# Nashatyrev/shadow

Hardware: AMD Instinct MI355X
Metric: APSP wall time + source-SSSPs/sec, 10k-vertex GML graph, 1/2/4/8 MI355X (higher is better)
Workload: dtype u32+f32

## Files before the change

include/shadow_routing.h:

```cpp
#ifndef SHADOW_ROUTING_H
#define SHADOW_ROUTING_H

#include <stddef.h>
#include <stdint.h>

#ifdef __cplusplus
extern "C" {
#endif

#define SRG_OK 0
#define SRG_ERR_ARG 1
#define SRG_ERR_NO_EDGE 2
#define SRG_ERR_MULTI_EDGE 3
#define SRG_ERR_UNREACHABLE 4
#define SRG_ERR_LATENCY_RANGE 5
#define SRG_ERR_HIP 6
#define SRG_ERR_OOM 7
#define SRG_ERR_PARSE 8
#define SRG_ERR_RCCL 9
#define SRG_ERR_INTERNAL 10

typedef struct srg_edge_list {
    uint32_t num_vertices;
    uint32_t directed;
// ... 66 lines not shown
#define SRG_OPT_SIMULATE_RANK 6
#define SRG_OPT_FW_TILE 7
#define SRG_OPT_SPARSE_DELTA_DIV 12
#define SRG_OPT_SPARSE_GLOBAL_BITMAPS 14
#define SRG_OPT_FW_SYMMETRIC 17
#define SRG_OPT_D2H_MODE 20
#define SRG_OPT_LOSS_CHUNKS 21
#define SRG_OPT_SCAN_GROUPS 22
#define SRG_OPT_H2D_CODEC 25
#define SRG_OPT_EDGE_SHARD 29
#define SRG_OPT_LATE_LOSS 30
#define SRG_OPT_FW_LINE_SPLIT 31
#define SRG_OPT_FW_STEP 32
#define SRG_OPT_FW_OVERLAP 33
#define SRG_OPT_TEST_FAULT 34
#define SRG_OPT_TABLE_POOL_BYTES 35
#define SRG_OPT_TABLE_POOL_IDLE_BYTES 36
#define SRG_OPT_CREATE_MS_RUNTIME 37
#define SRG_OPT_CREATE_MS_LIBRARY 38
#define SRG_OPT_FW_XCD_ORDER 39
#define SRG_OPT_SCAN_MIRROR 40
#define SRG_OPT_SCAN_MIRRORED 41
#define SRG_OPT_SCAN_MIRROR_CAP 42
int srg_set_option(srg_ctx* ctx, int option, double value);
int srg_get_option(srg_ctx* ctx, int option, double* value);

int srg_compute_shortest_paths(srg_ctx* ctx, const srg_edge_list* graph,
                               const uint32_t* nodes, uint32_t num_nodes,
                               uint64_t* out_latency_ns, float* out_packet_loss,
                               srg_stats* stats, char* errbuf, size_t errlen);

int srg_compute_shortest_paths_device(srg_ctx* ctx, const srg_edge_list* graph_dev,
                                      const uint32_t* nodes_dev, uint32_t num_nodes,
                                      uint64_t* out_latency_ns_dev, float* out_packet_loss_dev,
                                      void* hip_stream, srg_stats* stats,
                                      char* errbuf, size_t errlen);

int srg_get_direct_paths(srg_ctx* ctx, const srg_edge_list* graph,
                         const uint32_t* nodes, uint32_t num_nodes,
                         uint64_t* out_latency_ns, float* out_packet_loss,
                         srg_stats* stats, char* errbuf, size_t errlen);

typedef struct srg_routing_info srg_routing_info;
int srg_routing_info_build(srg_ctx* ctx, const srg_edge_list* graph, const uint32_t* gml_ids, uint32_t num_ids,
                           int use_shortest_paths, srg_routing_info** out, srg_stats* stats,
                           char* errbuf, size_t errlen);
// ... 89 lines not shown
```

shadow_amd/_native.py:

```python
import ctypes
import os

_HERE = os.path.dirname(os.path.abspath(__file__))
LIB_PATH = os.path.join(_HERE, "libshadow_routing.so")

SRG_OK = 0
SRG_ERR_ARG = 1
SRG_ERR_NO_EDGE = 2
SRG_ERR_MULTI_EDGE = 3
SRG_ERR_UNREACHABLE = 4
SRG_ERR_LATENCY_RANGE = 5
SRG_ERR_HIP = 6
SRG_ERR_OOM = 7
SRG_ERR_PARSE = 8
SRG_ERR_RCCL = 9
SRG_ERR_INTERNAL = 10
SRG_ERR_EVENT_ORDER = 11

SRG_PATH_DENSE_U32 = 0
SRG_PATH_DENSE_U64 = 1
SRG_PATH_DIRECT = 2
SRG_PATH_SPARSE_U32 = 3
SRG_PATH_SPARSE_U64 = 4

# ... 5 lines not shown
SRG_OPT_SIMULATE_RANK = 6
SRG_OPT_FW_TILE = 7
SRG_OPT_SPARSE_DELTA_DIV = 12
SRG_OPT_SPARSE_GLOBAL_BITMAPS = 14
SRG_OPT_FW_SYMMETRIC = 17
SRG_OPT_D2H_MODE = 20
SRG_OPT_LOSS_CHUNKS = 21
SRG_OPT_SCAN_GROUPS = 22
SRG_OPT_H2D_CODEC = 25
SRG_OPT_EDGE_SHARD = 29
SRG_OPT_LATE_LOSS = 30
SRG_OPT_FW_LINE_SPLIT = 31
SRG_OPT_FW_STEP = 32
SRG_OPT_FW_OVERLAP = 33
SRG_OPT_TEST_FAULT = 34
SRG_OPT_TABLE_POOL_BYTES = 35
SRG_OPT_TABLE_POOL_IDLE_BYTES = 36
SRG_OPT_CREATE_MS_RUNTIME = 37
SRG_OPT_CREATE_MS_LIBRARY = 38
SRG_OPT_FW_XCD_ORDER = 39
SRG_OPT_SCAN_MIRROR = 40
SRG_OPT_SCAN_MIRRORED = 41
SRG_OPT_SCAN_MIRROR_CAP = 42
SRG_ALGO_AUTO = 0
SRG_ALGO_DENSE = 1
SRG_ALGO_SPARSE = 2
SRG_UNIQUE_ID_BYTES = 128

SRG_SCAN_NONE = 0
SRG_SCAN_SPARSE = 1
SRG_SCAN_DENSE = 2

_u32p = ctypes.POINTER(ctypes.c_uint32)
_u64p = ctypes.POINTER(ctypes.c_uint64)
_f32p = ctypes.POINTER(ctypes.c_float)


class EdgeList(ctypes.Structure):
    _fields_ = [
        ("num_vertices", ctypes.c_uint32),
        ("directed", ctypes.c_uint32),
        ("num_edges", ctypes.c_uint64),
        ("src", ctypes.c_void_p),
        ("dst", ctypes.c_void_p),
        ("latency_ns", ctypes.c_void_p),
        ("packet_loss", ctypes.c_void_p),
# ... 197 lines not shown
```

shadow_amd/csrc/dense.hip.h:

```cpp
template <class K, int T>
bool run_dense(srg_ctx& c, const DevGraph& g, const Plan& pl, const uint32_t* nodes, uint32_t n, uint64_t* out_lat,
               float* out_loss, hipStream_t st, const Prelude& P, srg_stats* stats, HostSink* sink,
               FwOverlap* ov = nullptr) {
    const bool pre = ov && ov->on && ov->ok && ov->ended && sizeof(K) == 4 && T == FwOverlap::T;
    if (sizeof(K) == 8 && c.kout_key) {
        if (!(sink && sink->widen)) fail(SRG_INTERNAL_NEED_U64, "the build needs u64 latency keys: no u32 key table");
        sink->widen = false;
        c.kout_key = nullptr;
        c.kout_diag = nullptr;
    }
    const uint32_t V = g.V;
    const size_t Vp = ((size_t)V + T - 1) / T * T;
    const size_t VV = Vp * Vp;
    const bool multi = c.comm && c.comm->nranks > 1;
    Timer tm(st);
    c.own_row0 = pl.p0;
    c.own_row1 = pl.p1;

    K* W = (K*)c.b_W.get(VV * sizeof(K));
    uint32_t* WL = (uint32_t*)c.b_WL.get(VV * 4);
    K* D = (K*)c.b_D.get(VV * sizeof(K));
    bool wl_late = false;
    if (pre) {
        wl_late = g.late && !g.late->applied;
// ... 285 lines not shown
            HIP_CHECK(hipEventRecord(c.ev_dst, ax));
        }
        const size_t Eb = E_layout + 256;
        uint32_t* cscpos = (uint32_t*)c.b_cscfill.get((size_t)nbTT5 * nK5 * V5_TT * 4);
        K* ent_w = (K*)c.b_entw.get(Eb * sizeof(K));
        uint2* ent_ub = (uint2*)c.b_grpe.get(Eb * 8);
        uint32_t* cscent = (uint32_t*)c.b_cscent.get(std::max<uint64_t>(E_ess, 1) * 4);
        k_v5_cscpos<<<(NT + 255) / 256, 256, 0, st>>>(v5_cnt, cscoff, NT, nK5, cscpos);
        uint2* rec = (uint2*)c.b_entkey.get((Eb + V5_SLACK) * 8);
        {
            const size_t nwaves = (size_t)nw64 * nK5;
            k_v5_fill<K><<<(unsigned)((nwaves * 64 + 255) / 256), 256, 0, st>>>(ess, W, WL, Vp, V, nw64, nK5, v5_cnt,
                                                                                  v5_goff, cscpos, rec, ent_w,
                                                                                  ent_ub, cscent);
        }
        HIP_CHECK(hipGetLastError());
        const size_t lds_rows = loss_rows_lds(V);
        bool mirror = c.scan_mirror && !g.directed && pl.G == 1 && !multi && !simulated && nloc == n && P.ident &&
                      !v5lo && lds_rows <= 150 * 1024;
        const uint32_t scan_groups = c.scan_groups ? (uint32_t)c.scan_groups : mirror ? 4u : 3u;
        const bool interleave = sink_rows && lds_rows <= 150 * 1024 && scan_groups > 1;
        if (interleave) set_lds(k_loss_rows<K, true>, lds_rows);
        uint32_t* PREDK = lds_rows <= 150 * 1024 ? (uint32_t*)c.b_PRED2.get(nmax * Vp * 8) : nullptr;
        auto pack_pred = [&](uint32_t r0, uint32_t r1) {
            const uint32_t nsb = (r1 - r0 + 127) / 128, nt8 = (nbTT5 + 7) / 8;
            k_pred_pack<<<8u * nt8 * nsb, 256, 0, st>>>(PRED, Vp, r0, r1, NT, nbTT5, nsb, ent_ub, (uint2*)PREDK,
                                                        multi_cnt, mirror ? 1u : 0u);
            HIP_CHECK(hipGetLastError());
        };
        auto mirror_rows = [&](uint32_t r0, uint32_t r1) {
            if (r1 <= r0 || r1 <= SB) return;
            const size_t pairs = (size_t)(r1 - r0) * Vp, room = std::min<size_t>(pairs / 2, (size_t)1 << 30);
            const uint32_t cap = (uint32_t)std::min<size_t>(
                room, c.scan_mirror_cap ? (size_t)c.scan_mirror_cap : std::max<size_t>(pairs / 1024, 256));
            uint2* work = (uint2*)(PRED + (size_t)r0 * Vp);
            HIP_CHECK(hipMemsetAsync(mirror_cnt, 0, 4, st));
            const uint32_t nlow = (r1 - 1) / SB * SB;
            k_pred_mirror<<<dim3(nlow / 64, (r1 - r0 + 63) / 64), 256, 0, st>>>((uint2*)PREDK, Vp, r0, r1, V, work, cap,
                                                                               mirror_cnt, multi_cnt);
            k_mirror_slow<K><<<1024, 256, 0, st>>>(work, mirror_cnt, cap, DST, npad, ent_ub, ent_w, cscoff, cscent,
                                                   (uint2*)PREDK, Vp, multi_cnt);
            HIP_CHECK(hipGetLastError());
        };
        std::vector<uint32_t> tri_h;
        if (nloc) HIP_CHECK(hipStreamWaitEvent(st, c.ev_dst, 0));
        for (bool again = nloc != 0; again;) {
            again = false;
            if (interleave) HIP_CHECK(hipMemsetAsync(&P.flags->changed, 0, 4, st));
            const uint32_t inf_check = v5lo ? 0u : 1u;
            const uint32_t nbS5 = (uint32_t)(npad / SB);
            const uint32_t ng = interleave ? std::min<uint32_t>(scan_groups, nbS5) : 1u;
            auto cut = [&](uint32_t q) { return mirror ? scan_group_cut_tri(q, ng, nbS5) : scan_group_cut(q, ng, nbS5); };
            const uint32_t* tri_d = nullptr;
            std::vector<size_t> tri_off(ng + 1, 0);
            if (mirror) {
                tri_h.clear();
                for (uint32_t gi = 0; gi < ng; ++gi) {
                    tri_scan_blocks(cut(gi), cut(gi + 1), nbTT5, tri_h);
                    tri_off[gi + 1] = tri_h.size();
                }
                uint32_t* d = (uint32_t*)c.b_tri.get(std::max<size_t>(tri_h.size(), 1) * 4);
                if (!tri_h.empty()) HIP_CHECK(hipMemcpyAsync(d, tri_h.data(), tri_h.size() * 4, hipMemcpyHostToDevice, st));
                HIP_CHECK(hipMemsetAsync(mirror_cnt, 0, 8, st));
                tri_d = d;
            }
            for (uint32_t gi = 0; gi < ng; ++gi) {
                const uint32_t c0 = cut(gi), c1 = cut(gi + 1);
                if (c1 == c0) continue;
                const uint32_t nblk = mirror ? (uint32_t)(tri_off[gi + 1] - tri_off[gi])
                                             : (nbTT5 + 3) / 4 * ((c1 - c0 + 7) / 8);
                if (nblk)
                    tight_v5<<<8u * 32u * ((nblk + 7) / 8), V5_WAVES * 64, 0, st>>>(
                        DSTs, npad, dsts_bytes, lnodes, nloc, V, NT, nbTT5, c1, nK5, c0, v5_goff,
                        (const uint32_t*)c.b_entkey.get(0), PRED, Vp, inf_check, mirror ? tri_d + tri_off[gi] : nullptr);
                HIP_CHECK(hipGetLastError());
                if (interleave) {
                    const uint32_t r0 = c0 * SB, r1 = std::min<uint32_t>(c1 * SB, nloc);
                    if (r1 <= r0) continue;
                    pack_pred(r0, r1);
                    if (mirror) mirror_rows(r0, r1);
                    k_loss_rows<K, true><<<r1 - r0, 1024, lds_rows, st>>>(PREDK, Vp, V, lnodes, nloc, ent_ub, ent_w,
                                                                   DST, npad, cscoff, cscent, P.selfloss, nodes, n,
                                                                   lpos, out_loss, &P.flags->changed, r0,
                                                                   mirror ? mirror_cnt + 1 : nullptr);
                    HIP_CHECK(hipGetLastError());
                    sink->send_rows(st, out_loss, sink->loss, pl.p0 + r0, r1 - r0, 4);
                }
            }
            if (!PREDK) k_count_multi<<<nloc, kThreads, 0, st>>>(PRED, nloc, V, Vp, multi_cnt);
            HIP_CHECK(hipGetLastError());
            ms_scan += tm.lap();
            if (interleave) {
                sink->loss_sent = true;
                rb_async(c, MS_CHANGED, &P.flags->changed, st);
                if (mirror) rb_async(c, MS_MIRROR, mirror_cnt + 1, st);
                HIP_CHECK(hipStreamSynchronize(st));
                rounds = (int)rb_get<uint32_t>(c, MS_CHANGED);
                loss_written = true;
            } else if (lds_rows <= 150 * 1024) {
                set_lds(k_loss_rows<K, true>, lds_rows);
                HIP_CHECK(hipMemsetAsync(&P.flags->changed, 0, 4, st));
                pack_pred(0, nloc);
                if (mirror) mirror_rows(0, nloc);
                const uint32_t nchunk = std::max<uint32_t>(1, std::min<uint32_t>(c.loss_chunks ? c.loss_chunks : sink_rows ? 8 : 1, nloc));
                for (uint32_t q = 0; q < nchunk; ++q) {
                    const uint32_t r0 = (uint32_t)((uint64_t)nloc * q / nchunk);
                    const uint32_t r1 = (uint32_t)((uint64_t)nloc * (q + 1) / nchunk);
                    if (r1 == r0) continue;
                    k_loss_rows<K, true><<<r1 - r0, 1024, lds_rows, st>>>(PREDK, Vp, V, lnodes, nloc, ent_ub, ent_w,
                                                                   DST, npad, cscoff, cscent, P.selfloss, nodes, n,
                                                                   lpos, out_loss, &P.flags->changed, r0,
                                                                   mirror ? mirror_cnt + 1 : nullptr);
                    HIP_CHECK(hipGetLastError());
                    if (sink_rows) sink->send_rows(st, out_loss, sink->loss, pl.p0 + r0, r1 - r0, 4);
                }
                if (sink_rows) sink->loss_sent = true;
                rb_async(c, MS_CHANGED, &P.flags->changed, st);
                if (mirror) rb_async(c, MS_MIRROR, mirror_cnt + 1, st);
                HIP_CHECK(hipStreamSynchronize(st));
                rounds = (int)rb_get<uint32_t>(c, MS_CHANGED);
                loss_written = true;
            } else {
                float* L0 = (float*)c.b_L0.get(nmax * Vp * 4);
                float* L1 = (float*)c.b_L1.get(nmax * Vp * 4);
                k_fill<float><<<grid_for((size_t)nloc * Vp), kThreads, 0, st>>>(L0, (size_t)nloc * Vp, 1.0f);
// ... 102 lines not shown
```

shadow_amd/csrc/env_switches.h:

```cpp
#pragma once
#include <algorithm>
#include <cstddef>
#include <cstdlib>
#include <cstring>

namespace srg_env {

static inline bool is_set(const char* name) { return std::getenv(name) != nullptr; }
static inline bool first_char_is(const char* name, char ch) {
    const char* e = std::getenv(name);
    return e && e[0] == ch;
}
static inline bool equals(const char* name, const char* value) {
    const char* e = std::getenv(name);
    return e && std::strcmp(e, value) == 0;
}

static inline bool stream_hops_events() { return equals("SRG_STREAM_HOPS", "events"); }
static inline int fw_bulk_q() {
    const char* e = std::getenv("SRG_FW_BULK_Q");
    return !e ? -1 : e[0] == '0' ? 0 : e[0] == '1' ? 1 : -1;
}
static inline bool debug_overlap() { return is_set("SRG_DEBUG_OVERLAP"); }
static inline int debug_sparse() {
    const char* e = std::getenv("SRG_DEBUG_SPARSE");
    return !e ? 0 : e[0] == '2' ? 2 : 1;
}
static inline bool debug_codec() { return is_set("SRG_DEBUG_CODEC"); }
static inline bool debug_create() { return is_set("SRG_DEBUG_CREATE"); }
static inline bool sparse_kernel_bf() { return equals("SRG_SPARSE_KERNEL", "bf"); }
static inline bool sparse_split_off() { return first_char_is("SRG_SPARSE_SPLIT", '0'); }
static inline bool latency_unit_ns() { return equals("SRG_LATENCY_UNIT", "1"); }
static inline int codec_threads() {
    const char* e = std::getenv("SRG_CODEC_THREADS");
    return e ? std::max(1, std::atoi(e)) : 0;
}
static inline bool codec_seq_off() { return equals("SRG_CODEC_SEQ", "0"); }
static inline bool codec_slow_after(size_t& chunk) {
    const char* e = std::getenv("SRG_CODEC_SLOW_AFTER");
    if (e) chunk = (size_t)std::atoll(e);
    return e != nullptr;
}
static inline bool prefault_on() { return !equals("SRG_PREFAULT", "0"); }
static inline bool no_key_d2h() { return is_set("SRG_NO_KEY_D2H"); }
static inline bool create_warm_off() { return first_char_is("SRG_CREATE_WARM", '0'); }

}
```

shadow_amd/csrc/plan.h:

```cpp
#pragma once
#include <algorithm>
#include <cstddef>
#include <cstdint>
#include <vector>

namespace {

struct Plan {
    int G = 1, g = 0, nb = 0, rb0 = 0, rb1 = 0;
    std::vector<int> blk_lo;
    uint32_t p0 = 0, p1 = 0;
    std::vector<uint32_t> lnodes, lpos;
    int owner(int b) const { return (int)(std::upper_bound(blk_lo.begin(), blk_lo.end(), b) - blk_lo.begin()) - 1; }
    bool own(int b) const { return b >= rb0 && b < rb1; }
};

inline void tri_tile_h(int nb, int idx, int& I, int& J) {
    int i = 0;
    while (i + 1 < nb && (i + 1) * nb - (i + 1) * i / 2 <= idx) ++i;
    I = i;
    J = i + (idx - (i * nb - i * (i - 1) / 2));
}

inline Plan make_plan(int G, int g, uint32_t V, int T, const std::vector<uint32_t>& nodes_h) {
// ... 64 lines not shown
        for (uint32_t sg = 0; c0 + 8 * sg < c1; ++sg)
            for (uint32_t tb = 0; 4 * tb < ntiles; ++tb)
                if (std::min(4 * tb + 3, ntiles - 1) >= c0 + 8 * sg) out.push_back(tb | sg << 16);
    while ((out.size() - base) % 8) out.push_back(TRI_PAD);
}

inline uint64_t tri_scan_work(uint32_t c, uint32_t nblocks) { return (uint64_t)c * nblocks - (uint64_t)c * (c ? c - 1 : 0) / 2; }
inline uint32_t scan_group_cut_tri(uint32_t q, uint32_t ng, uint32_t nblocks) {
    if (q == 0) return 0u;
    if (q >= ng) return nblocks;
    const uint32_t last = nblocks ? (nblocks - 1) / 8 * 8 : 0u;
    const bool tail = ng >= 3 && last > 0;
    const uint32_t end = tail ? last : nblocks;
    const uint32_t parts = tail ? ng - 1 : ng;
    if (q >= parts) return end;
    const uint64_t want = tri_scan_work(end, nblocks) / 2;
    uint32_t c = 0;
    while (c < end && tri_scan_work(c, nblocks) < want) ++c;
    const uint32_t half = std::min(end, (c + 4) / 8 * 8);
    if (q == 1) return half;
    return std::min(end, half + ((end - half) * (q - 1) / (parts - 1) + 4) / 8 * 8);
}

}
```

shadow_amd/csrc/routing.hip:

```cpp
#include <hip/hip_runtime.h>
#include <hsa/hsa.h>
#include <hsa/hsa_ext_amd.h>
#include <sys/mman.h>

#include <algorithm>
#include <atomic>
#include <chrono>
#include <cmath>
#include <condition_variable>
#include <deque>
#include <cstdio>
#include <cstdlib>
#include <cstring>
#include <functional>
#include <map>
#include <memory>
#include <mutex>
#include <new>
#include <stdexcept>
#include <string>
#include <thread>
#include <vector>

#include "../../include/shadow_routing.h"
// ... 705 lines not shown
    DevBuf b_cflags, b_tiles, b_tslot;
    uint32_t* fw_timeout = nullptr;
    unsigned char* hbox = nullptr;
    uint32_t* sig[2] = {nullptr, nullptr};
    uint32_t sig_val[2] = {0, 0};
    bool hop_values = false;
    unsigned long long hop_bound_ticks = 200000000ull;
    Event ev_fwreset;
    Event ev_dst;
    int fw_line_split = 0;
    int fw_step = -1;
    DevBuf b_xlb, b_xflags;
    uint32_t xepoch = 0;
    std::vector<Event> ev_ov;
    uint32_t* kout_key = nullptr;
    uint64_t* kout_diag = nullptr;
    DevBuf b_odiag;
    int fw_overlap = 1;
    int fw_xcd_order = 1;
    int scan_mirror = 1;
    int scan_mirrored = 0;
    int scan_mirror_cap = 0;
    DevBuf b_tri;
    int test_fault = 0;
    std::shared_ptr<TablePool> tpool = std::make_shared<TablePool>();
    double ms_create_runtime = 0, ms_create_lib = 0;
    DevBuf b_ek0, b_ek1, b_eh0, b_eh1, b_ei0, b_ei1, b_ehist, b_eoffs, b_ered;
    ~srg_ctx() {
        delete comm;
        for (uint32_t* p : sig)
            if (p) (void)hipFree(p);
        if (h_lring) (void)hipHostFree(h_lring);
        if (hbox) (void)hipHostFree(hbox);
        for (hipStream_t s : {aux_stream, comm_stream, d2h_stream, stream})
            if (s) (void)hipStreamDestroy(s);
        delete pool;
        if (h_ring) (void)hipHostFree(h_ring);
        tpool->close();
    }
};

namespace {

struct LateLoss {
    hipStream_t ls = nullptr;
    std::thread th;
// ... 1068 lines not shown
            begun = true;
        }
        while (next < nb && (next + 1 < nb ? A >= next + 1 : A >= nb - 1)) {
            fw->pivot(next, A);
            if (dbg) pe.push_back(tev(st));
            ++next;
        }
        if (next == nb && !ended) {
            fw->end(ms_xchg);
            ended = true;
        }
    }
};

#include "dense.hip.h"
#include "sparse_run.hip.h"

void compute_device(srg_ctx& c, const DevGraph& g, const uint32_t* nodes, uint32_t n, uint64_t* out_lat,
                    float* out_loss, hipStream_t st, srg_stats* stats, HostSink* sink = nullptr,
                    FwOverlap* ov = nullptr) {
    HIP_CHECK(hipStreamSynchronize(c.aux_stream));
    HIP_CHECK(hipStreamSynchronize(c.comm_stream));
    c.scan_mirrored = 0;
    if (g.V == 0) {
        if (n) fail(SRG_ERR_ARG, "nodes given for an empty graph");
        return;
    }
    const bool ov_fw = ov && ov->on && ov->ok && ov->begun;
    Prelude P = prelude(c, g, nodes, n, ov_fw ? c.comm_stream : st, true);
    if (n == 0) return;
    const uint64_t unit = (P.es.unit > 1 && !srg_env::latency_unit_ns()) ? P.es.unit : 1;
    P.unit = unit;
    const bool pre = ov && ov->on && ov->ok && ov->ended && P.es.max_lat < 0xFFFFFFFFull;
    if (pre) P.unit = 1;
    P.max_key = P.es.max_lat / P.unit;
    if (stats) stats->latency_unit_ns = P.unit;
    const unsigned __int128 bound = (unsigned __int128)P.max_key * (g.V > 1 ? g.V - 1 : 1);
    P.range_risk = bound >= ((unsigned __int128)1 << 62);
    P.wrap_risk = (unsigned __int128)P.es.max_lat * g.V >= ((unsigned __int128)1 << 64);
    const int G = c.comm ? c.comm->nranks : 1, rk = c.comm ? c.comm->rank : 0;
    if (choose_sparse(c, g) && !P.wrap_risk) {
        loss_arrive(g, P.selfloss, st);
        if (P.max_key < 0xFFFFFFFFull && run_sparse(c, g, nodes, n, out_lat, out_loss, st, P, stats)) return;
        run_sparse(c, g, nodes, n, out_lat, out_loss, st, P, stats, true);
        return;
    }
// ... 1008 lines not shown
        case SRG_OPT_FW_OVERLAP:
            if (value != 0 && value != 1) return SRG_ERR_ARG;
            ctx->fw_overlap = (int)value;
            return SRG_OK;
        case SRG_OPT_TEST_FAULT:
            if (value != 0 && value != 1 && value != 2) return SRG_ERR_ARG;
#ifndef SRG_TEST_HOOKS
            if (value != 0) return SRG_ERR_ARG;
#endif
            ctx->test_fault = (int)value;
            return SRG_OK;
        case SRG_OPT_FW_XCD_ORDER:
            if (value != 0 && value != 1) return SRG_ERR_ARG;
            ctx->fw_xcd_order = (int)value;
            return SRG_OK;
        case SRG_OPT_SCAN_MIRROR:
            if (value != 0 && value != 1) return SRG_ERR_ARG;
            ctx->scan_mirror = (int)value;
            return SRG_OK;
        case SRG_OPT_SCAN_MIRROR_CAP:
            if (!(value >= 0 && value <= 1073741824.0)) return SRG_ERR_ARG;
            ctx->scan_mirror_cap = (int)value;
            return SRG_OK;
        case SRG_OPT_TABLE_POOL_BYTES: {
            if (!(value >= 0.0 && value <= 1e15)) return SRG_ERR_ARG;
            std::lock_guard<std::mutex> pl(ctx->tpool->mu);
            ctx->tpool->limit = (size_t)value;
            ctx->tpool->max_idle = 0;
            ctx->tpool->trim_locked(ctx->tpool->limit);
            return SRG_OK;
        }
        case SRG_OPT_ALGORITHM:
            if (value != SRG_ALGO_AUTO && value != SRG_ALGO_DENSE && value != SRG_ALGO_SPARSE) return SRG_ERR_ARG;
            ctx->algorithm = (int)value;
            return SRG_OK;
        default:
            return SRG_ERR_ARG;
    }
}

int srg_get_option(srg_ctx* ctx, int option, double* value) {
    if (!ctx || !value) return SRG_ERR_ARG;
    std::lock_guard<std::mutex> lk(ctx->mu);
    switch (option) {
        case SRG_OPT_PROFILING: *value = ctx->profiling; break;
        case SRG_OPT_SPARSE_THRESHOLD: *value = ctx->sparse_threshold; break;
// ... 10 lines not shown
        case SRG_OPT_H2D_CODEC: *value = ctx->h2d_codec; break;
        case SRG_OPT_EDGE_SHARD: *value = ctx->edge_shard; break;
        case SRG_OPT_LATE_LOSS: *value = ctx->late_loss; break;
        case SRG_OPT_FW_LINE_SPLIT: *value = ctx->fw_line_split; break;
        case SRG_OPT_FW_STEP: *value = ctx->fw_step; break;
        case SRG_OPT_FW_OVERLAP: *value = ctx->fw_overlap; break;
        case SRG_OPT_TEST_FAULT: *value = ctx->test_fault; break;
        case SRG_OPT_TABLE_POOL_BYTES: {
            std::lock_guard<std::mutex> pl(ctx->tpool->mu);
            *value = (double)ctx->tpool->limit;
            break;
        }
        case SRG_OPT_TABLE_POOL_IDLE_BYTES: {
            std::lock_guard<std::mutex> pl(ctx->tpool->mu);
            *value = (double)ctx->tpool->idle_bytes;
            break;
        }
        case SRG_OPT_CREATE_MS_RUNTIME: *value = ctx->ms_create_runtime; break;
        case SRG_OPT_FW_XCD_ORDER: *value = ctx->fw_xcd_order; break;
        case SRG_OPT_CREATE_MS_LIBRARY: *value = ctx->ms_create_lib; break;
        case SRG_OPT_SCAN_MIRROR: *value = ctx->scan_mirror; break;
        case SRG_OPT_SCAN_MIRRORED: *value = ctx->scan_mirrored; break;
        case SRG_OPT_SCAN_MIRROR_CAP: *value = ctx->scan_mirror_cap; break;
        default: return SRG_ERR_ARG;
    }
    return SRG_OK;
}

void srg_destroy(srg_ctx* ctx) {
    if (!ctx) return;
    (void)hipSetDevice(ctx->device);
    {
        std::lock_guard<std::mutex> lk(g_dev_mu);
        --g_dev_ctx[ctx->device];
    }
    delete ctx;
}

int srg_internal_compute_table(srg_ctx* ctx, const srg_edge_list* graph, const uint32_t* nodes, uint32_t num_nodes,
                               int shortest, uint64_t* out_lat, uint32_t* out_key, uint64_t* out_diag, float* out_loss,
                               uint64_t* unit_ns, srg_table* tab_lat, srg_table* tab_loss, srg_stats* stats,
                               char* errbuf, size_t errlen) {
    srg_stats local{};
    srg_stats* st = stats ? stats : &local;
    srg_table* tabs[2] = {tab_lat, tab_loss};
    const int rc = host_entry(ctx, graph, nodes, num_nodes, out_key ? nullptr : out_lat, out_loss, st, errbuf, errlen,
// ... 375 lines not shown
```

shadow_amd/csrc/tight_sparse.hip.h:

```cpp
#pragma once
#include <hip/hip_runtime.h>
#include <stdint.h>

#include "kernels.hip.h"

namespace srg {

template <class K>
__global__ void __launch_bounds__(256) k_ess_mask(const K* __restrict__ W, const K* __restrict__ D, size_t ld,
                                                   uint32_t V, uint32_t u0, uint32_t u1, uint32_t nw64,
                                                   unsigned long long* __restrict__ ess) {
    const uint32_t lane = threadIdx.x & 63, wave = threadIdx.x >> 6;
    const uint32_t u = u0 + blockIdx.x;
    if (u >= u1) return;
    const K* Wu = W + (size_t)u * ld;
    const K* Du = D + (size_t)u * ld;
    unsigned long long* eu = ess + (size_t)u * nw64;
    if constexpr (sizeof(K) == 4) {
        for (uint32_t w0 = wave * 4; w0 < nw64; w0 += 16) {
            const uint32_t t = w0 * 64 + lane * 4;
            uint4 a = make_uint4(0u, 0u, 0u, 0u), d = make_uint4(1u, 1u, 1u, 1u);
            if (t < ld) {
                a = *reinterpret_cast<const uint4*>(Wu + t);
                d = *reinterpret_cast<const uint4*>(Du + t);
// ... 132 lines not shown
            ++e;
        }
    }
    if (c & 1u) {
        rec[e] = make_uint2(0u, KeyOps<uint32_t>::INF);
        ent_w[e] = KeyOps<K>::INF;
        ent_ub[e] = make_uint2(0u, __float_as_uint(1.0f));
    }
    if (j == V5_TW - 1) {
        const uint32_t total = incl;
        for (size_t q = 2 * ((size_t)pbase + total); q < 2 * (size_t)goff[g + 1]; ++q) {
            rec[q] = make_uint2(0u, KeyOps<uint32_t>::INF);
            ent_w[q] = KeyOps<K>::INF;
            ent_ub[q] = make_uint2(0u, __float_as_uint(1.0f));
        }
    }
}

typedef uint32_t v16u_v5 __attribute__((ext_vector_type(16)));
struct alignas(64) V5Grp {
    uint32_t v[16];
};

__global__ void __launch_bounds__(512, 4) tight_v5(const uint32_t* __restrict__ DST, size_t npad, uint32_t dst_bytes,
                                                    const uint32_t* __restrict__ nodes, uint32_t n, uint32_t V,
                                                    uint32_t NT, uint32_t nbTT, uint32_t nbS, uint32_t nK, uint32_t c0,
                                                    const uint32_t* __restrict__ goff, const uint32_t* __restrict__ rec,
                                                    uint32_t* __restrict__ PRED, size_t ldp, uint32_t inf_check,
                                                    const uint32_t* __restrict__ tri) {
    __shared__ __attribute__((aligned(16))) uint32_t rows[2 * V5_UC * V5_SB];
    const uint32_t bid = blockIdx.x, xcd = bid & 7, slot = bid >> 3;
    const uint32_t blk = (slot >> 5) * 8 + xcd, nbb = (nbTT + 3) / 4;
    uint32_t tb = blk % nbb, sg = blk / nbb;
    if (tri) {
        const uint32_t d = tri[blk];
        if (d == 0xFFFFFFFFu) return;
        tb = d & 0xFFFFu;
        sg = d >> 16;
    }
    const uint32_t b = tb * 4 + (slot & 3), c = c0 + sg * 8 + ((slot >> 2) & 7);
    if (c >= nbS || b >= nbTT) return;
    if (tri && b < c) return;
    const uint32_t tid = threadIdx.x, lane = tid & 63;
    const uint32_t wave = (uint32_t)__builtin_amdgcn_readfirstlane(tid >> 6);
    const uint32_t r0 = c * V5_SB + 2 * lane;
    const __amdgpu_buffer_rsrc_t rsrc = make_rsrc(DST, dst_bytes);
    const uint32_t t0 = b * V5_TT + wave * V5_TW;
    const bool active = t0 < NT;
    v16u_v5 ndl, ndh, stl, sth;
#pragma unroll
    for (uint32_t j = 0; j < V5_TW; ++j) {
        uint32_t dl = 0, dh = 0;
        if (active) {
            const auto v = __builtin_amdgcn_raw_buffer_load_b64(rsrc, ((t0 + j) * (uint32_t)npad + r0) * 4u, 0, 0);
            dl = v[0];
            dh = v[1];
        }
        ndl[j] = 0u - dl;
        ndh[j] = 0u - dh;
        stl[j] = PRED_NONE;
        sth[j] = PRED_NONE;
    }
    const uint32_t srow = tid >> 5, scol = (tid & 31) * 4;
    uint4 sv[4];
    auto stage_load = [&](uint32_t k) {
#pragma unroll
        for (uint32_t i = 0; i < 4; ++i) {
            const uint32_t u = k * V5_UC + srow + 16 * i;
            const auto v = __builtin_amdgcn_raw_buffer_load_b128(rsrc, (u * (uint32_t)npad + c * V5_SB + scol) * 4u, 0, 0);
            sv[i] = make_uint4(v[0], v[1], v[2], v[3]);
        }
    };
    auto stage_store = [&](uint32_t buf) {
#pragma unroll
        for (uint32_t i = 0; i < 4; ++i)
            *reinterpret_cast<uint4*>(&rows[buf * (V5_UC * V5_SB) + (srow + 16 * i) * V5_SB + scol]) = sv[i];
    };
    stage_load(0);
    stage_store(0);
    __syncthreads();
    const unsigned char* lds = reinterpret_cast<const unsigned char*>(rows);
    for (uint32_t k = 0; k < nK; ++k) {
        if (k + 1 < nK) stage_load(k + 1);
        if (active) {
            const size_t q = ((size_t)b * nK + k) * V5_WAVES + wave;
            const uint32_t p0 = (uint32_t)__builtin_amdgcn_readfirstlane(goff[q]);
            const uint32_t p1 = (uint32_t)__builtin_amdgcn_readfirstlane(goff[q + 1]);
            const uint32_t vb = (k & 1u) * (V5_UC * V5_SB * 4u) + lane * 8u;
            auto group = [&](const V5Grp& cur, uint32_t p) {
                    uint2 A[8];
#pragma unroll
                    for (uint32_t i = 0; i < 4; ++i) {
                        A[2 * i] = *reinterpret_cast<const uint2*>(lds + vb + (cur.v[4 * i] & 0xFFFFu));
                        A[2 * i + 1] = *reinterpret_cast<const uint2*>(lds + vb + cur.v[4 * i + 2]);
                    }
#pragma unroll
                    for (uint32_t i = 0; i < 4; ++i) {
                        const uint32_t tl = cur.v[4 * i] >> 16;
                        const uint32_t dl = ndl[tl], dh = ndh[tl];
                        const uint32_t w0 = cur.v[4 * i + 1], w1 = cur.v[4 * i + 3];
                        const uint32_t x0l = A[2 * i].x + w0 + dl, x0h = A[2 * i].y + w0 + dh;
                        const uint32_t x1l = A[2 * i + 1].x + w1 + dl, x1h = A[2 * i + 1].y + w1 + dh;
                        const uint32_t m = min(min(x0l, x0h), min(x1l, x1h));
                        if (__builtin_expect(__ballot(m == 0) != 0, 0)) {
                            const uint32_t e0 = 2 * (p + i);
                            uint32_t sl = stl[tl], sh = sth[tl];
                            if (x0l == 0) sl = (sl == PRED_NONE) ? e0 : PRED_MULTI;
                            if (x1l == 0) sl = (sl == PRED_NONE) ? e0 + 1 : PRED_MULTI;
                            if (x0h == 0) sh = (sh == PRED_NONE) ? e0 : PRED_MULTI;
                            if (x1h == 0) sh = (sh == PRED_NONE) ? e0 + 1 : PRED_MULTI;
                            stl[tl] = sl;
                            sth[tl] = sh;
                        }
                    }
            };
            if (p0 < p1) {
                V5Grp ga = *reinterpret_cast<const V5Grp*>(rec + 4 * (size_t)p0);
                V5Grp gb = *reinterpret_cast<const V5Grp*>(rec + 4 * (size_t)(p0 + 4));
                for (uint32_t p = p0;; p += 8) {
                    group(ga, p);
                    if (p + 4 >= p1) break;
                    ga = *reinterpret_cast<const V5Grp*>(rec + 4 * (size_t)(p + 8));
                    group(gb, p + 4);
                    if (p + 8 >= p1) break;
                    gb = *reinterpret_cast<const V5Grp*>(rec + 4 * (size_t)(p + 12));
                }
            }
        }
        if (k + 1 < nK) {
            stage_store((k + 1) & 1u);
            __syncthreads();
        }
    }
    if (!active) return;
#pragma unroll
    for (uint32_t h = 0; h < 2; ++h) {
        const uint32_t r = r0 + h;
        if (r >= n) continue;
        const uint32_t s = nodes[r];
        uint32_t o[V5_TW];
#pragma unroll
        for (uint32_t j = 0; j < V5_TW; ++j) {
            const uint32_t t = t0 + j;
            const uint32_t nd = h ? ndh[j] : ndl[j];
            const uint32_t st = h ? sth[j] : stl[j];
            o[j] = (t >= V || t == s || (inf_check && nd == 0u - KeyOps<uint32_t>::INF)) ? PRED_NONE : st;
        }
        uint4* out = reinterpret_cast<uint4*>(PRED + (size_t)r * ldp + t0);
#pragma unroll
        for (uint32_t j = 0; j < V5_TW; j += 4) out[j / 4] = make_uint4(o[j], o[j + 1], o[j + 2], o[j + 3]);
    }
}

__global__ void __launch_bounds__(256) k_pred_pack(const uint32_t* __restrict__ PRED, size_t ldp, uint32_t r0,
                                                   uint32_t r1, uint32_t NT, uint32_t nbTT, uint32_t nsb,
                                                   const uint2* __restrict__ ent_ub, uint2* __restrict__ PK,
                                                   unsigned long long* __restrict__ multi, uint32_t tri) {
    const uint32_t xcd = blockIdx.x & 7, slot = blockIdx.x >> 3;
    const uint32_t b = xcd + 8 * (slot / nsb), sb = slot % nsb;
    if (b >= nbTT) return;
    if (tri && b < r0 / V5_SB + sb) return;
    const uint32_t tx = threadIdx.x & 31, ty = threadIdx.x >> 5;
    const uint32_t t = b * V5_TT + tx * 4;
    const bool tv = t < NT;
    uint32_t nm = 0;
    for (uint32_t i0 = ty; i0 < 128; i0 += 32) {
        uint32_t pv[4][4];
#pragma unroll
        for (int k = 0; k < 4; ++k) {
            const uint32_t r = r0 + sb * 128 + i0 + 8 * k;
            uint4 p = make_uint4(PRED_NONE, PRED_NONE, PRED_NONE, PRED_NONE);
            if (tv && r < r1) p = *reinterpret_cast<const uint4*>(PRED + (size_t)r * ldp + t);
            pv[k][0] = p.x;
            pv[k][1] = p.y;
            pv[k][2] = p.z;
            pv[k][3] = p.w;
        }
        uint2 q[4][4];
#pragma unroll
        for (int k = 0; k < 4; ++k)
#pragma unroll
            for (int j = 0; j < 4; ++j) {
                q[k][j] = pv[k][j] < PRED_MULTI ? ent_ub[pv[k][j]] : make_uint2(pv[k][j], 0u);
                nm += pv[k][j] == PRED_MULTI;
            }
#pragma unroll
        for (int k = 0; k < 4; ++k) {
            const uint32_t r = r0 + sb * 128 + i0 + 8 * k;
            if (!tv || r >= r1) break;
            uint4* o = reinterpret_cast<uint4*>(PK + (size_t)r * ldp + t);
            o[0] = make_uint4(q[k][0].x, q[k][0].y, q[k][1].x, q[k][1].y);
            o[1] = make_uint4(q[k][2].x, q[k][2].y, q[k][3].x, q[k][3].y);
        }
    }
    if (__ballot(nm != 0)) {
#pragma unroll
        for (int o = 32; o > 0; o >>= 1) nm += __shfl_xor(nm, o, 64);
        if ((threadIdx.x & 63) == 0) atomicAdd(multi, (unsigned long long)nm);
    }
}

constexpr uint32_t MIRROR_STEPS = 64;
__global__ void __launch_bounds__(256) k_pred_mirror(uint2* __restrict__ PK, size_t ldp, uint32_t r0, uint32_t r1,
                                                     uint32_t V, uint2* __restrict__ work, uint32_t cap,
                                                     uint32_t* __restrict__ wcnt,
                                                     unsigned long long* __restrict__ multi) {
    __shared__ uint2 tile[64][65];
    __shared__ uint32_t overflowed;
    const uint32_t tt = r0 / 64 + blockIdx.y, sc = blockIdx.x * 64;
    if (sc >= tt / 2 * V5_SB) return;
    if (threadIdx.x == 0) overflowed = wcnt[1];
    __syncthreads();
    if (overflowed) return;
    const uint32_t lane = threadIdx.x & 63, wave = threadIdx.x >> 6;
    const uint32_t t = tt * 64 + lane;
    uint32_t nm = 0;
    for (uint32_t i = 0; i < 16; ++i) {
        const uint32_t sl = wave * 16 + i, s = sc + sl, bs = s / V5_SB;
        uint2 res = make_uint2(PRED_NONE, 0u);
        if (t < r1) {
            const uint2* rs = PK + (size_t)s * ldp;
// ... 248 lines not shown
```

Before: 233,500.

## Split scan over K chunks with XCD-balanced work lists and predecessor merge

Replaces the fixed scan block indexing (and the triangular block list) with a host-built work list. The list can split each tile's K range into up to 8 pieces and deals the pieces greedily across the 8 XCDs to balance load. A cost model picks the split factor automatically by default. Partial predecessor planes go to an extra buffer and are merged either during pred packing or by a new merge kernel. This aims to fix XCD imbalance and tail underuse, at the cost of extra memory traffic, merge work and host planning time.

```diff
diff --git a/include/shadow_routing.h b/include/shadow_routing.h
--- a/include/shadow_routing.h
+++ b/include/shadow_routing.h
@@ -112,6 +112,8 @@
 #define SRG_OPT_SCAN_MIRROR 40
 #define SRG_OPT_SCAN_MIRRORED 41
 #define SRG_OPT_SCAN_MIRROR_CAP 42
+#define SRG_OPT_SCAN_SPLIT 43
+#define SRG_OPT_SCAN_SPLIT_USED 44
 int srg_set_option(srg_ctx* ctx, int option, double value);
 int srg_get_option(srg_ctx* ctx, int option, double* value);
 
diff --git a/shadow_amd/_native.py b/shadow_amd/_native.py
--- a/shadow_amd/_native.py
+++ b/shadow_amd/_native.py
@@ -51,6 +51,8 @@
 SRG_OPT_SCAN_MIRROR = 40
 SRG_OPT_SCAN_MIRRORED = 41
 SRG_OPT_SCAN_MIRROR_CAP = 42
+SRG_OPT_SCAN_SPLIT = 43
+SRG_OPT_SCAN_SPLIT_USED = 44
 SRG_ALGO_AUTO = 0
 SRG_ALGO_DENSE = 1
 SRG_ALGO_SPARSE = 2
diff --git a/shadow_amd/csrc/dense.hip.h b/shadow_amd/csrc/dense.hip.h
--- a/shadow_amd/csrc/dense.hip.h
+++ b/shadow_amd/csrc/dense.hip.h
@@ -331,10 +331,11 @@
         const bool interleave = sink_rows && lds_rows <= 150 * 1024 && scan_groups > 1;
         if (interleave) set_lds(k_loss_rows<K, true>, lds_rows);
         uint32_t* PREDK = lds_rows <= 150 * 1024 ? (uint32_t*)c.b_PRED2.get(nmax * Vp * 8) : nullptr;
-        auto pack_pred = [&](uint32_t r0, uint32_t r1) {
+        uint32_t* PREDX = nullptr;
+        auto pack_pred = [&](uint32_t r0, uint32_t r1, uint32_t Q, size_t pstride) {
             const uint32_t nsb = (r1 - r0 + 127) / 128, nt8 = (nbTT5 + 7) / 8;
             k_pred_pack<<<8u * nt8 * nsb, 256, 0, st>>>(PRED, Vp, r0, r1, NT, nbTT5, nsb, ent_ub, (uint2*)PREDK,
-                                                        multi_cnt, mirror ? 1u : 0u);
+                                                        multi_cnt, mirror ? 1u : 0u, Q, PREDX, pstride);
             HIP_CHECK(hipGetLastError());
         };
         auto mirror_rows = [&](uint32_t r0, uint32_t r1) {
@@ -351,7 +352,10 @@
                                                    (uint2*)PREDK, Vp, multi_cnt);
             HIP_CHECK(hipGetLastError());
         };
-        std::vector<uint32_t> tri_h;
+        std::vector<ScanItem> plan_h;
+        const int env_split = srg_env::scan_split();
+        const uint32_t scan_split = (uint32_t)(env_split >= 0 ? env_split : c.scan_split);
+        if (nK5 > 0xFFFFu || (nbTT5 + 3) / 4 > 0xFFFFu) fail(SRG_ERR_INTERNAL, "the scan's work list holds 16-bit chunk and tile indices");
         if (nloc) HIP_CHECK(hipStreamWaitEvent(st, c.ev_dst, 0));
         for (bool again = nloc != 0; again;) {
             again = false;
@@ -360,33 +364,37 @@
             const uint32_t nbS5 = (uint32_t)(npad / SB);
             const uint32_t ng = interleave ? std::min<uint32_t>(scan_groups, nbS5) : 1u;
             auto cut = [&](uint32_t q) { return mirror ? scan_group_cut_tri(q, ng, nbS5) : scan_group_cut(q, ng, nbS5); };
-            const uint32_t* tri_d = nullptr;
-            std::vector<size_t> tri_off(ng + 1, 0);
-            if (mirror) {
-                tri_h.clear();
-                for (uint32_t gi = 0; gi < ng; ++gi) {
-                    tri_scan_blocks(cut(gi), cut(gi + 1), nbTT5, tri_h);
-                    tri_off[gi + 1] = tri_h.size();
-                }
-                uint32_t* d = (uint32_t*)c.b_tri.get(std::max<size_t>(tri_h.size(), 1) * 4);
-                if (!tri_h.empty()) HIP_CHECK(hipMemcpyAsync(d, tri_h.data(), tri_h.size() * 4, hipMemcpyHostToDevice, st));
-                HIP_CHECK(hipMemsetAsync(mirror_cnt, 0, 8, st));
-                tri_d = d;
-            }
+            std::vector<size_t> plan_off(ng + 1, 0), plan_stride(ng, 0);
+            std::vector<uint32_t> plan_q(ng, 1u);
+            plan_h.clear();
+            size_t px_words = 0;
+            for (uint32_t gi = 0; gi < ng; ++gi) {
+                const uint32_t c0 = cut(gi), c1 = cut(gi + 1);
+                plan_q[gi] = scan_plan(c0, c1, nbTT5, nK5, mirror, scan_split, plan_h);
+                plan_off[gi + 1] = plan_h.size();
+                plan_stride[gi] = (size_t)(c1 - c0) * SB * Vp;
+                px_words = std::max(px_words, (plan_q[gi] - 1) * plan_stride[gi]);
+                if (c1 > c0) c.scan_split_used = std::max(c.scan_split_used, (int)plan_q[gi]);
+            }
+            const uint2* plan_d = (const uint2*)c.b_tri.get(std::max<size_t>(plan_h.size(), 1) * sizeof(ScanItem));
+            if (!plan_h.empty())
+                HIP_CHECK(hipMemcpyAsync((void*)plan_d, plan_h.data(), plan_h.size() * sizeof(ScanItem), hipMemcpyHostToDevice, st));
+            PREDX = px_words ? (uint32_t*)c.b_PREDX.get(px_words * 4) : nullptr;
+            if (mirror) HIP_CHECK(hipMemsetAsync(mirror_cnt, 0, 8, st));
             for (uint32_t gi = 0; gi < ng; ++gi) {
                 const uint32_t c0 = cut(gi), c1 = cut(gi + 1);
                 if (c1 == c0) continue;
-                const uint32_t nblk = mirror ? (uint32_t)(tri_off[gi + 1] - tri_off[gi])
-                                             : (nbTT5 + 3) / 4 * ((c1 - c0 + 7) / 8);
-                if (nblk)
-                    tight_v5<<<8u * 32u * ((nblk + 7) / 8), V5_WAVES * 64, 0, st>>>(
+                const uint32_t nlist = (uint32_t)(plan_off[gi + 1] - plan_off[gi]);
+                if (nlist)
+                    tight_v5<<<32u * nlist, V5_WAVES * 64, 0, st>>>(
                         DSTs, npad, dsts_bytes, lnodes, nloc, V, NT, nbTT5, c1, nK5, c0, v5_goff,
-                        (const uint32_t*)c.b_entkey.get(0), PRED, Vp, inf_check, mirror ? tri_d + tri_off[gi] : nullptr);
+                        (const uint32_t*)c.b_entkey.get(0), PRED, Vp, inf_check, plan_d + plan_off[gi], mirror ? 1u : 0u,
+                        plan_q[gi], PREDX, plan_stride[gi]);
                 HIP_CHECK(hipGetLastError());
                 if (interleave) {
                     const uint32_t r0 = c0 * SB, r1 = std::min<uint32_t>(c1 * SB, nloc);
                     if (r1 <= r0) continue;
-                    pack_pred(r0, r1);
+                    pack_pred(r0, r1, plan_q[gi], plan_stride[gi]);
                     if (mirror) mirror_rows(r0, r1);
                     k_loss_rows<K, true><<<r1 - r0, 1024, lds_rows, st>>>(PREDK, Vp, V, lnodes, nloc, ent_ub, ent_w,
                                                                    DST, npad, cscoff, cscent, P.selfloss, nodes, n,
@@ -396,7 +404,12 @@
                     sink->send_rows(st, out_loss, sink->loss, pl.p0 + r0, r1 - r0, 4);
                 }
             }
-            if (!PREDK) k_count_multi<<<nloc, kThreads, 0, st>>>(PRED, nloc, V, Vp, multi_cnt);
+            if (!PREDK) {
+                if (plan_q[0] > 1)
+                    k_pred_merge<<<grid_for((size_t)nloc * (NT / 4), 256 * 64), kThreads, 0, st>>>(PRED, Vp, 0u, nloc, NT, plan_q[0],
+                                                                                                  PREDX, plan_stride[0]);
+                k_count_multi<<<nloc, kThreads, 0, st>>>(PRED, nloc, V, Vp, multi_cnt);
+            }
             HIP_CHECK(hipGetLastError());
             ms_scan += tm.lap();
             if (interleave) {
@@ -409,7 +422,7 @@
             } else if (lds_rows <= 150 * 1024) {
                 set_lds(k_loss_rows<K, true>, lds_rows);
                 HIP_CHECK(hipMemsetAsync(&P.flags->changed, 0, 4, st));
-                pack_pred(0, nloc);
+                pack_pred(0, nloc, plan_q[0], plan_stride[0]);
                 if (mirror) mirror_rows(0, nloc);
                 const uint32_t nchunk = std::max<uint32_t>(1, std::min<uint32_t>(c.loss_chunks ? c.loss_chunks : sink_rows ? 8 : 1, nloc));
                 for (uint32_t q = 0; q < nchunk; ++q) {
diff --git a/shadow_amd/csrc/env_switches.h b/shadow_amd/csrc/env_switches.h
--- a/shadow_amd/csrc/env_switches.h
+++ b/shadow_amd/csrc/env_switches.h
@@ -44,5 +44,10 @@
 static inline bool prefault_on() { return !equals("SRG_PREFAULT", "0"); }
 static inline bool no_key_d2h() { return is_set("SRG_NO_KEY_D2H"); }
 static inline bool create_warm_off() { return first_char_is("SRG_CREATE_WARM", '0'); }
+static inline int scan_split() {
+    const char* e = std::getenv("SRG_SCAN_SPLIT");
+    if (!e || !e[0] || e[1]) return -1;
+    return e[0] == '0' || e[0] == '1' || e[0] == '2' || e[0] == '4' || e[0] == '8' ? e[0] - '0' : -1;
+}
 
 }
diff --git a/shadow_amd/csrc/plan.h b/shadow_amd/csrc/plan.h
--- a/shadow_amd/csrc/plan.h
+++ b/shadow_amd/csrc/plan.h
@@ -110,4 +110,83 @@
     return std::min(end, half + ((end - half) * (q - 1) / (parts - 1) + 4) / 8 * 8);
 }
 
+struct ScanItem {
+    uint32_t blk, k;
+};
+constexpr double SCAN_SPLIT_OVH = 0.05;
+constexpr uint32_t SCAN_XCDS = 8, SCAN_XCD_SLOTS = 64;
+
+inline uint32_t scan_piece_k(uint32_t q, uint32_t Q, uint32_t nK) { return (uint32_t)((uint64_t)q * nK / Q); }
+inline uint32_t scan_split_clamp(uint32_t Q, uint32_t nK) { return std::max(1u, std::min(Q, nK)); }
+
+inline uint32_t scan_block_live(uint32_t tb, uint32_t sg, uint32_t c0, uint32_t c1, uint32_t ntiles, bool tri) {
+    uint32_t live = 0;
+    for (uint32_t slot = 0; slot < 32; ++slot) {
+        const uint32_t b = tb * 4 + (slot & 3), c = c0 + sg * 8 + ((slot >> 2) & 7);
+        live += b < ntiles && c < c1 && (!tri || b >= c);
+    }
+    return live;
 }
+
+inline uint32_t scan_deal(uint32_t c0, uint32_t c1, uint32_t ntiles, uint32_t nK, bool tri, uint32_t Q,
+                          std::vector<ScanItem>* out) {
+    struct Piece {
+        uint64_t w;
+        uint32_t live;
+        ScanItem d;
+    };
+    std::vector<Piece> pieces;
+    if (ntiles && nK && c1 > c0)
+        for (uint32_t sg = 0; c0 + 8 * sg < c1; ++sg)
+            for (uint32_t tb = 0; 4 * tb < ntiles; ++tb) {
+                const uint32_t live = scan_block_live(tb, sg, c0, c1, ntiles, tri);
+                if (!live) continue;
+                for (uint32_t q = 0; q < Q; ++q) {
+                    const uint32_t k0 = scan_piece_k(q, Q, nK), k1 = scan_piece_k(q + 1, Q, nK);
+                    pieces.push_back({(uint64_t)live * (k1 - k0), live, {tb | sg << 16, k0 | k1 << 16}});
+                }
+            }
+    std::stable_sort(pieces.begin(), pieces.end(), [](const Piece& a, const Piece& b) { return a.w > b.w; });
+    uint64_t load[SCAN_XCDS] = {};
+    uint32_t items[SCAN_XCDS] = {};
+    std::vector<ScanItem> lists[SCAN_XCDS];
+    for (const Piece& p : pieces) {
+        uint32_t x = 0;
+        for (uint32_t i = 1; i < SCAN_XCDS; ++i)
+            if (load[i] < load[x]) x = i;
+        load[x] += p.w;
+        items[x] += p.live;
+        if (out) lists[x].push_back(p.d);
+    }
+    if (out) {
+        size_t len = 0;
+        for (const auto& l : lists) len = std::max(len, l.size());
+        for (size_t i = 0; i < len; ++i)
+            for (uint32_t x = 0; x < SCAN_XCDS; ++x) out->push_back(i < lists[x].size() ? lists[x][i] : ScanItem{TRI_PAD, 0u});
+    }
+    return *std::max_element(items, items + SCAN_XCDS);
+}
+
+inline double scan_model_cost(uint32_t busiest, uint32_t Q, double ovh = SCAN_SPLIT_OVH) {
+    return (double)((busiest + SCAN_XCD_SLOTS - 1) / SCAN_XCD_SLOTS) * (1.0 / Q + ovh);
+}
+
+inline uint32_t scan_plan(uint32_t c0, uint32_t c1, uint32_t ntiles, uint32_t nK, bool tri, uint32_t split,
+                          std::vector<ScanItem>& out, double ovh = SCAN_SPLIT_OVH) {
+    uint32_t Q = scan_split_clamp(split, nK);
+    if (!split) {
+        double best = 0;
+        for (uint32_t cand : {1u, 2u, 4u, 8u}) {
+            const uint32_t q = scan_split_clamp(cand, nK);
+            const double cost = scan_model_cost(scan_deal(c0, c1, ntiles, nK, tri, q, nullptr), q, ovh);
+            if (cand == 1 || cost < best) {
+                best = cost;
+                Q = q;
+            }
+        }
+    }
+    scan_deal(c0, c1, ntiles, nK, tri, Q, &out);
+    return Q;
+}
+
+}
diff --git a/shadow_amd/csrc/routing.hip b/shadow_amd/csrc/routing.hip
--- a/shadow_amd/csrc/routing.hip
+++ b/shadow_amd/csrc/routing.hip
@@ -751,6 +751,9 @@
     int scan_mirrored = 0;
     int scan_mirror_cap = 0;
     DevBuf b_tri;
+    int scan_split = 0;
+    int scan_split_used = 0;
+    DevBuf b_PREDX;
     int test_fault = 0;
     std::shared_ptr<TablePool> tpool = std::make_shared<TablePool>();
     double ms_create_runtime = 0, ms_create_lib = 0;
@@ -1865,6 +1868,7 @@
     HIP_CHECK(hipStreamSynchronize(c.aux_stream));
     HIP_CHECK(hipStreamSynchronize(c.comm_stream));
     c.scan_mirrored = 0;
+    c.scan_split_used = 0;
     if (g.V == 0) {
         if (n) fail(SRG_ERR_ARG, "nodes given for an empty graph");
         return;
@@ -2919,6 +2923,10 @@
             if (!(value >= 0 && value <= 1073741824.0)) return SRG_ERR_ARG;
             ctx->scan_mirror_cap = (int)value;
             return SRG_OK;
+        case SRG_OPT_SCAN_SPLIT:
+            if (value != 0 && value != 1 && value != 2 && value != 4 && value != 8) return SRG_ERR_ARG;
+            ctx->scan_split = (int)value;
+            return SRG_OK;
         case SRG_OPT_TABLE_POOL_BYTES: {
             if (!(value >= 0.0 && value <= 1e15)) return SRG_ERR_ARG;
             std::lock_guard<std::mutex> pl(ctx->tpool->mu);
@@ -2975,6 +2983,8 @@
         case SRG_OPT_SCAN_MIRROR: *value = ctx->scan_mirror; break;
         case SRG_OPT_SCAN_MIRRORED: *value = ctx->scan_mirrored; break;
         case SRG_OPT_SCAN_MIRROR_CAP: *value = ctx->scan_mirror_cap; break;
+        case SRG_OPT_SCAN_SPLIT: *value = ctx->scan_split; break;
+        case SRG_OPT_SCAN_SPLIT_USED: *value = ctx->scan_split_used; break;
         default: return SRG_ERR_ARG;
     }
     return SRG_OK;
diff --git a/shadow_amd/csrc/tight_sparse.hip.h b/shadow_amd/csrc/tight_sparse.hip.h
--- a/shadow_amd/csrc/tight_sparse.hip.h
+++ b/shadow_amd/csrc/tight_sparse.hip.h
@@ -178,22 +178,22 @@
     uint32_t v[16];
 };
 
+__device__ __forceinline__ uint32_t pred_merge(uint32_t a, uint32_t b) {
+    return a == PRED_NONE ? b : b == PRED_NONE ? a : PRED_MULTI;
+}
+
 __global__ void __launch_bounds__(512, 4) tight_v5(const uint32_t* __restrict__ DST, size_t npad, uint32_t dst_bytes,
                                                     const uint32_t* __restrict__ nodes, uint32_t n, uint32_t V,
                                                     uint32_t NT, uint32_t nbTT, uint32_t nbS, uint32_t nK, uint32_t c0,
                                                     const uint32_t* __restrict__ goff, const uint32_t* __restrict__ rec,
                                                     uint32_t* __restrict__ PRED, size_t ldp, uint32_t inf_check,
-                                                    const uint32_t* __restrict__ tri) {
+                                                    const uint2* __restrict__ list, uint32_t tri, uint32_t Q,
+                                                    uint32_t* __restrict__ PX, size_t pstride) {
     __shared__ __attribute__((aligned(16))) uint32_t rows[2 * V5_UC * V5_SB];
     const uint32_t bid = blockIdx.x, xcd = bid & 7, slot = bid >> 3;
-    const uint32_t blk = (slot >> 5) * 8 + xcd, nbb = (nbTT + 3) / 4;
-    uint32_t tb = blk % nbb, sg = blk / nbb;
-    if (tri) {
-        const uint32_t d = tri[blk];
-        if (d == 0xFFFFFFFFu) return;
-        tb = d & 0xFFFFu;
-        sg = d >> 16;
-    }
+    const uint2 d = list[(slot >> 5) * 8 + xcd];
+    if (d.x == 0xFFFFFFFFu) return;
+    const uint32_t tb = d.x & 0xFFFFu, sg = d.x >> 16, k0 = d.y & 0xFFFFu, k1 = d.y >> 16;
     const uint32_t b = tb * 4 + (slot & 3), c = c0 + sg * 8 + ((slot >> 2) & 7);
     if (c >= nbS || b >= nbTT) return;
     if (tri && b < c) return;
@@ -232,12 +232,12 @@
         for (uint32_t i = 0; i < 4; ++i)
             *reinterpret_cast<uint4*>(&rows[buf * (V5_UC * V5_SB) + (srow + 16 * i) * V5_SB + scol]) = sv[i];
     };
-    stage_load(0);
-    stage_store(0);
+    stage_load(k0);
+    stage_store(k0 & 1u);
     __syncthreads();
     const unsigned char* lds = reinterpret_cast<const unsigned char*>(rows);
-    for (uint32_t k = 0; k < nK; ++k) {
-        if (k + 1 < nK) stage_load(k + 1);
+    for (uint32_t k = k0; k < k1; ++k) {
+        if (k + 1 < k1) stage_load(k + 1);
         if (active) {
             const size_t q = ((size_t)b * nK + k) * V5_WAVES + wave;
             const uint32_t p0 = (uint32_t)__builtin_amdgcn_readfirstlane(goff[q]);
@@ -283,12 +283,15 @@
                 }
             }
         }
-        if (k + 1 < nK) {
+        if (k + 1 < k1) {
             stage_store((k + 1) & 1u);
             __syncthreads();
         }
     }
     if (!active) return;
+    const uint32_t q = Q > 1 ? (uint32_t)(((uint64_t)k0 * Q + nK - 1) / nK) : 0u;
+    uint32_t* plane = q ? PX + (size_t)(q - 1) * pstride : PRED;
+    const uint32_t prow0 = q ? c0 * V5_SB : 0u;
 #pragma unroll
     for (uint32_t h = 0; h < 2; ++h) {
         const uint32_t r = r0 + h;
@@ -302,7 +305,7 @@
             const uint32_t st = h ? sth[j] : stl[j];
             o[j] = (t >= V || t == s || (inf_check && nd == 0u - KeyOps<uint32_t>::INF)) ? PRED_NONE : st;
         }
-        uint4* out = reinterpret_cast<uint4*>(PRED + (size_t)r * ldp + t0);
+        uint4* out = reinterpret_cast<uint4*>(plane + (size_t)(r - prow0) * ldp + t0);
 #pragma unroll
         for (uint32_t j = 0; j < V5_TW; j += 4) out[j / 4] = make_uint4(o[j], o[j + 1], o[j + 2], o[j + 3]);
     }
@@ -311,7 +314,8 @@
 __global__ void __launch_bounds__(256) k_pred_pack(const uint32_t* __restrict__ PRED, size_t ldp, uint32_t r0,
                                                    uint32_t r1, uint32_t NT, uint32_t nbTT, uint32_t nsb,
                                                    const uint2* __restrict__ ent_ub, uint2* __restrict__ PK,
-                                                   unsigned long long* __restrict__ multi, uint32_t tri) {
+                                                   unsigned long long* __restrict__ multi, uint32_t tri,
+                                                   uint32_t Q, const uint32_t* __restrict__ PX, size_t pstride) {
     const uint32_t xcd = blockIdx.x & 7, slot = blockIdx.x >> 3;
     const uint32_t b = xcd + 8 * (slot / nsb), sb = slot % nsb;
     if (b >= nbTT) return;
@@ -326,7 +330,13 @@
         for (int k = 0; k < 4; ++k) {
             const uint32_t r = r0 + sb * 128 + i0 + 8 * k;
             uint4 p = make_uint4(PRED_NONE, PRED_NONE, PRED_NONE, PRED_NONE);
-            if (tv && r < r1) p = *reinterpret_cast<const uint4*>(PRED + (size_t)r * ldp + t);
+            if (tv && r < r1) {
+                p = *reinterpret_cast<const uint4*>(PRED + (size_t)r * ldp + t);
+                for (uint32_t q = 1; q < Q; ++q) {
+                    const uint4 x = *reinterpret_cast<const uint4*>(PX + (size_t)(q - 1) * pstride + (size_t)(r - r0) * ldp + t);
+                    p = make_uint4(pred_merge(p.x, x.x), pred_merge(p.y, x.y), pred_merge(p.z, x.z), pred_merge(p.w, x.w));
+                }
+            }
             pv[k][0] = p.x;
             pv[k][1] = p.y;
             pv[k][2] = p.z;
@@ -353,6 +363,22 @@
 #pragma unroll
         for (int o = 32; o > 0; o >>= 1) nm += __shfl_xor(nm, o, 64);
         if ((threadIdx.x & 63) == 0) atomicAdd(multi, (unsigned long long)nm);
+    }
+}
+
+__global__ void __launch_bounds__(256) k_pred_merge(uint32_t* __restrict__ PRED, size_t ldp, uint32_t r0, uint32_t r1,
+                                                    uint32_t NT, uint32_t Q, const uint32_t* __restrict__ PX,
+                                                    size_t pstride) {
+    const size_t per = NT / 4, total = (size_t)(r1 - r0) * per;
+    for (size_t i = blockIdx.x * (size_t)blockDim.x + threadIdx.x; i < total; i += (size_t)gridDim.x * blockDim.x) {
+        const size_t rr = i / per, t = (i - rr * per) * 4;
+        uint4* o = reinterpret_cast<uint4*>(PRED + (r0 + rr) * ldp + t);
+        uint4 p = *o;
+        for (uint32_t q = 1; q < Q; ++q) {
+            const uint4 x = *reinterpret_cast<const uint4*>(PX + (size_t)(q - 1) * pstride + rr * ldp + t);
+            p = make_uint4(pred_merge(p.x, x.x), pred_merge(p.y, x.y), pred_merge(p.z, x.z), pred_merge(p.w, x.w));
+        }
+        *o = p;
     }
 }
 
```

Result: slower. 227,100 (-2.7%).
